# kevlar-dev/kevlar

Hardware: AMD Instinct MI355X
Metric: reads/sec through count+novel (3 samples, k=31) (higher is better)
Workload: dtype u64 hash / u8 counters

## Files before the change

__graft_entry__.py:

```python
import os
import subprocess
import sys

ROOT = os.path.dirname(os.path.abspath(__file__))
CSRC = os.path.join(ROOT, 'kevlar_amd', 'csrc')
HIP_SOURCES = ['kv_host.hip', 'kv_fastx.hip', 'kv_kernels.hip', 'kv_binned.hip', 'kv_skm.hip', 'kv_novel.hip', 'kv_graph.hip', 'kv_shard.hip', 'kv_inflate.hip', 'kv_gunzip.hip', 'kv_fastq.hip', 'kv_augfastx.hip', 'kv_synth.hip']
HIP_HEADERS = ['kv_internal.h', 'kv_knobs.h', 'kv_fastmod.h', 'kv_device.h', 'kv_binned.h', 'kv_skm_device.h', 'kv_novel_device.h', 'kv_kmer2bit_device.h', 'kv_inflate_device.h',
               os.path.join('..', '..', 'include', 'kvsketch.h')]
LIB = os.path.join(ROOT, 'kevlar_amd', 'libkvsketch_hip.so')


def _stale(target, deps):
    if not os.path.exists(target):
        return True
    t = os.path.getmtime(target)
    return any(os.path.getmtime(d) > t for d in deps)


def _compile(srcs, headers, lib, force=False, extra=()):
    from concurrent.futures import ThreadPoolExecutor
    hipcc = os.environ.get('HIPCC', '/opt/rocm/bin/hipcc')
    tag = ''.join(c if c.isalnum() else '_' for c in ' '.join(extra))
    objdir = os.path.join(CSRC, 'build', tag or 'default')
    os.makedirs(objdir, exist_ok=True)
# ... 83 lines not shown
```

kevlar_amd/csrc/kv_host.hip:

```cpp
#include <algorithm>
#include <functional>
#include <atomic>
#include <cstdarg>
#include <map>

#include "kv_internal.h"

static thread_local char g_err[512] = "";
thread_local int kv_last_hip_code = 0;

void kv_set_error(const char *fmt, ...)
{
    va_list ap;
    va_start(ap, fmt);
    vsnprintf(g_err, sizeof(g_err), fmt, ap);
    va_end(ap);
}

uint64_t kv_next_uid()
{
    static std::atomic<uint64_t> next{1};
    return next.fetch_add(1);
}

// ... 1114 lines not shown
    {"KV_COUNT_PATH", T_, "atomic | binned | skm: pin the count path"},
    {"KV_NOVEL_PATH", T_, "tiles | skm: pin the scan path"},
    {"KV_ROUTE_PATH", T_, "plain: the exchange routes one item per k-mer (no combining)"},
    {"KV_SET_SCAN", T_, "skm: a shard's set scan keeps the bucketed kernel"},
    {"KV_BIN_2BIT", T_, "0: stage A never hashes from the 2-bit form"},
    {"KV_SKM_S2", T_, "plain | sorted: pin the fine split"},
    {"KV_SKM_ANY_K", T_, "use the kernels with k at run time, not the k = 31 / 51 instances"},
    {"KV_SKM_BUCKET_KMERS", T_, "k-mer occurrences aimed at per bucket (tests: many buckets on small inputs)"},
    {"KV_SKM_CAP_PCT", T_, "segment capacity in per cent of the estimate (tests: push records through the loose list)"},
    {"KV_SKM_LOOSE_CAP", T_, "entries of the loose list"},
    {"KV_SKM_FORCE_LOOSE", T_, "one key in 64 is counted as if its table were full: its occurrences travel through the loose list"},
    {"KV_SKM_DL", T_, "0: no distinct list from a case sample's count; 1: from the first batch on"},
    {"KV_SKM_NO_REUSE", T_, "the scan re-buckets the batch instead of reusing the count's buckets"},
    {"KV_NOVEL_2BIT", T_, "0: the per-k-mer scan keeps the tile kernel"},
    {"KV_NOVEL_BITS", T_, "0: no bit map as the first probe of the scan"},
    {"KV_NOVEL_BITS_MIN", T_, "items from which the pairs scan builds its bit map"},
    {"KV_NOVEL_PAIRS", T_, "0: the set scan answers from hashes alone"},
    {"KV_NOVEL_REREAD", T_, "`kevlar novel` reads a case file again for the scan instead of keeping its batch"},
    {"KV_HOST_SORT", T_, "partition sorts its keys on the host"},
    {"KV_STAGE", T_, "0: uploads straight from the file mapping, no pinned staging"},
    {"KV_INGEST_TEXT_MB", T_, "text per ingest batch in MB (tests: small batches)"},
    {"KV_GUNZIP_TEXT_MIN_MB", T_, "gzip files from this size on are inflated on the device"},
    {"KV_GUNZIP_CHUNK_KB", T_, "1..64: compressed bytes per probe stretch"},
    {"KV_MEX_PASSES", T_, "exchange: combine passes per bucket, at least (1-16)"},
    {"KV_MEX_DL_POOL", T_, "exchange: 1 = the owner's distinct list as a pool of chunks at once (it is the last resort of an owner short of memory)"},
    {"KV_MEX_PAIRS", T_, "9: (hash, count) pairs travel in the 9-byte block form"},
    {"KV_MEX_TEST_DECLINE", T_, "point:rank -- that rank fails at that point of the exchange (tests of the agreed fallbacks)"},
    {"KV_ALLBANDS_TEST_FAIL", T_, "rank:band -- `novel --all-bands`: that rank fails before counting that band (0-based; test of the agreed stop)"},
    {"KV_ROUTE_OVF_CAP", T_, "entries of the route's overflow list (tests: force the capacity error)"},
};
// ... 56 lines not shown
```

kevlar_amd/csrc/kv_internal.h:

```cpp
#pragma once
#include <hip/hip_runtime.h>

#include <cstdint>
#include <cstdio>
#include <cstdlib>
#include <cstring>
#include <functional>
#include <atomic>
#include <mutex>
#include <string>
#include <vector>
#include "kv_knobs.h"

#include "../../include/kvsketch.h"
#include "kv_fastmod.h"

enum { ST_BYTE = 0, ST_NIBBLE = 1, ST_BIT = 2 };
enum { HF_MURMUR = 0, HF_TWOBIT = 1 };

static inline int kv_storage_of(int kind)
{
    switch (kind) {
    case KV_COUNTTABLE: case KV_COUNTGRAPH: return ST_BYTE;
    case KV_SMALLCOUNTTABLE: case KV_SMALLCOUNTGRAPH: return ST_NIBBLE;
// ... 155 lines not shown
    uint64_t band_lo, band_hi;
    int use_mask, threshold, consume_masked;
};

bool kv_binned_eligible(const kv_sketch *s, const kv_reads *reads, uint64_t n_kmers, int nbands);
int kv_consume_binned(kv_sketch *s, const kv_reads *reads, const uint64_t *d_list, uint32_t list_stride,
                      const ConsumeFilter &filter, const kv_sketch *mask, uint64_t n_kmers, int nbands, uint64_t *n_added,
                      bool weighted_list = false);
double kv_estimate_distinct(uint64_t occupied, uint64_t size);

struct NovelParams;
bool kv_skm_eligible(const kv_sketch *s, const kv_reads *reads, uint64_t n_kmers, bool for_scan);
bool kv_skm_eligible_kind(int hashfam, int ksize, const kv_reads *reads, uint64_t n_kmers, bool for_scan);
int kv_consume_skm(kv_sketch *s, const kv_reads *reads, const ConsumeFilter &filter, const kv_sketch *mask,
                   uint64_t n_kmers, int nbands, uint64_t *n_added);
int kv_skm_novel_mark(const kv_reads *reads, const NovelParams &p, uint64_t n_kmers);
void kv_tile_hits_launch(const kv_reads *reads, const NovelParams &p, hipStream_t st);
bool kv_skm_list_ready(const kv_reads *reads, int ksize);

struct KvRouteSink {
    int ndest;
    uint32_t nwg;
    uint64_t bs;
    uint64_t seg_cap;
    uint64_t *seg;
    uint32_t *seg_count;
    uint64_t *ovf;
    uint8_t *ovf_dest;
    uint64_t ovf_cap;
    unsigned long long *ctr;
};
// ... 140 lines not shown
```

kevlar_amd/csrc/kv_novel.hip:

```cpp
#include <algorithm>
#include <functional>
#include <map>

#include "kv_binned.h"
#include "kv_novel_device.h"
#include "kv_kmer2bit_device.h"

namespace {

#define VC_WINDOW 3
#define VC_WINDOW_MAX 9
__device__ __forceinline__ uint32_t kmer_minimizer_key(const uint32_t *__restrict__ words, uint32_t pos, int k, int window)
{
    const uint32_t w0 = pos >> 4, sh = 2u * (pos & 15u);
    const uint64_t lo = (uint64_t)words[w0] | ((uint64_t)words[w0 + 1] << 32);
    uint64_t code = lo >> sh;
    if (sh) code |= (uint64_t)words[w0 + 2] << (64u - sh);
    const uint64_t kmask = k == 32 ? ~0ull : ((1ull << (2 * k)) - 1ull);
    code &= kmask;
    uint64_t rev = __brevll(code);
    rev = ((rev >> 1) & 0x5555555555555555ull) | ((rev & 0x5555555555555555ull) << 1);
    rev = (~rev >> (64 - 2 * k)) & kmask;
    const int m = k - (window - 1);
    const uint64_t mmask = (1ull << (2 * m)) - 1ull;
// ... 360 lines not shown
    load_descs(ns, p);
    __syncthreads();
    const int S = p.ncase + p.nctrl, k = p.hp.k;
    const uint32_t uni_wpr = (rd.uni_len + 15u) >> 4;
    for (uint64_t i = blockIdx.x * 256ull + threadIdx.x; i < nhits; i += (uint64_t)gridDim.x * 256ull) {
        const uint32_t read = p.hit_read[i], off = p.hit_off[i];
        const uint32_t *words = rd.words + (rd.uni_len ? (uint64_t)read * uni_wpr : rd.woff[read]);
        uint64_t bw[2] = {skm_bases32(words, off), KW == 2 ? skm_bases32(words, off + 32u) : 0ull};
        const SkmKey<KW> f = skm_first_kmer<KW>(bw, k);
        const uint64_t h = skm_key_hash<KW>(f, lut, p.hp);
        if (p.ab_keys && ab_lookup(p, h, p.hit_abund + i * (uint64_t)S, S)) continue;
        hit_abundances(ns, p, h, p.hit_abund + i * (uint64_t)S);
    }
}

struct VerdictCache {
    unsigned long long *p = nullptr;
    int bits = 0;
    uint64_t signature = 0;
};
std::map<hipStream_t, VerdictCache> g_vcache;
std::mutex g_vcache_mu;

struct DevBuf {
    void *p = nullptr;
    ~DevBuf() { if (p) (void)hipFree(p); }
    hipError_t alloc(size_t n) { return kv_hip_malloc(&p, n ? n : 4); }
    template <typename T> T *as() { return (T *)p; }
};

// ... 4 lines not shown
    {
        if (n <= bytes) return hipSuccess;
        if (p) (void)hipFree(p);
        p = nullptr; bytes = 0;
        hipError_t e = kv_hip_malloc(&p, n);
        if (e == hipSuccess) bytes = n;
        return e;
    }
};
struct ScanArenas {
    Arena work, hits, set, abund;
    std::mutex mu;
    hipStream_t copy_stream = nullptr;
    hipEvent_t kdone = nullptr, copied = nullptr;
    bool copy_pending = false;
};
thread_local bool g_hits_lazy = false;
std::map<hipStream_t, ScanArenas> g_scan_arenas;
std::mutex g_scan_arenas_mu;
inline size_t up256(size_t v) { return (v + 255) & ~(size_t)255; }

int attach_vcache(NovelParams &p, kv_sketch *const *ctrls, int ncase, int nctrl, int ctrl_max, uint64_t n_kmers, hipStream_t st)
{
    if (nctrl > 0 && p.screen == 0) {
        uint64_t sig = 0x9e3779b97f4a7c15ull ^ (uint64_t)(uint32_t)ctrl_max;
        for (int c = ncase; c < ncase + nctrl; ++c) {
            const kv_sketch *sk = ctrls[c - ncase];
            sig = (sig ^ sk->uid) * 0xff51afd7ed558ccdull;
            sig = (sig ^ sk->version) * 0xc4ceb9fe1a85ec53ull;
        }
// ... 122 lines not shown
    std::lock_guard<std::mutex> arena_lock(arenas->mu);
    hipError_t e = hipSuccess;
    if (arenas->copy_pending) {
        e = hipStreamWaitEvent(st, arenas->copied, 0);
        arenas->copy_pending = false;
    }
    const uint64_t mask_words = d_mask ? 0 : (reads->n_reads * min_stride + 31) / 32;
    if (mask_words * 4 > ((uint64_t)64 << 30)) {
        kv_set_error("kv_novel_scan: %llu reads with a longest read of %u bases need a %llu GB hit mask; "
                     "scan long sequences in a batch of their own", (unsigned long long)reads->n_reads, reads->max_len,
                     (unsigned long long)(mask_words * 4 >> 30));
        delete hits;
        *out = nullptr;
        return KV_ERR_CAPACITY;
    }
    const size_t b_mask = up256(mask_words * 4), b_flags = p.screen > 0 ? up256(reads->n_reads * 4) : 0;
    const size_t b_tcount = up256((uint64_t)reads->n_tiles * 4), b_tbase = up256(((uint64_t)reads->n_tiles + 1) * 8);
    e = arenas->work.need(b_mask + b_flags + b_tcount + b_tbase + 256);
    unsigned char *wp = (unsigned char *)arenas->work.p;
    if (e == hipSuccess) {
        if (d_mask) {
            p.mask = d_mask; p.mask_stride = mask_stride;
        } else {
            p.mask_stride = min_stride;
            p.mask = (uint32_t *)wp;
            e = hipMemsetAsync(p.mask, 0, mask_words * 4, st);
        }
        wp += b_mask;
    }
    if (e == hipSuccess && p.screen > 0) {
        p.disc_first = (uint32_t *)wp;
        e = hipMemsetAsync(p.disc_first, 0xFF, reads->n_reads * 4, st);
    }
    wp += b_flags;
    p.tile_count = (uint32_t *)wp; wp += b_tcount;
    uint64_t *d_tbase_p = (uint64_t *)wp;
    p.tile_base = d_tbase_p;
    uint64_t nhits = 0;
    bool marked_by_skm = use_skm;
    p.ab_keys = nullptr; p.ab_vals = nullptr; p.ab_mask = 0; p.ab_list = nullptr; p.ab_count = nullptr; p.ab_list_cap = 0;
    if (e == hipSuccess && use_skm && !p.set_keys && kv_skm_list_ready(reads, k)) {
        uint64_t slots = 1u << 16;
        while (slots < n_kmers / 64 && slots < (1ull << 24)) slots <<= 1;
        const uint64_t list_cap = slots / 8;
        if (arenas->abund.need(up256(slots * 8) + up256(slots * (uint64_t)S) + up256(list_cap * 4) + 256) == hipSuccess) {
            p.ab_keys = (unsigned long long *)arenas->abund.p;
            p.ab_vals = (uint8_t *)arenas->abund.p + up256(slots * 8);
            p.ab_mask = slots - 1;
            p.ab_list = (uint32_t *)(p.ab_vals + up256(slots * (uint64_t)S));
            p.ab_count = (unsigned int *)((unsigned char *)p.ab_list + up256(list_cap * 4));
            p.ab_list_cap = (uint32_t)list_cap;
            e = hipMemsetAsync(p.ab_keys, 0, slots * 8, st);
            if (e == hipSuccess) e = hipMemsetAsync(p.ab_count, 0, 4, st);
        } else {
            (void)hipGetLastError();
        }
    }
    if (e == hipSuccess && use_skm) {
        const int rc = kv_skm_novel_mark(reads, p, n_kmers);
        if (rc == KV_ERR_CAPACITY) {
            marked_by_skm = false;
            if (skm_overflowed) *skm_overflowed = true;
            const int rc2 = prepare_tile_scan();
            if (rc2 != KV_OK) { delete hits; *out = nullptr; return rc2; }
        } else if (rc != KV_OK) {
            delete hits;
            *out = nullptr;
            return rc;
        }
    }
    if (e == hipSuccess) {
        const char *forced = kv_knob("KV_NOVEL_PATH"), *nm2 = kv_knob("KV_NOVEL_2BIT");
        const bool two_bit = !marked_by_skm && p.screen == 0 && fam == HF_MURMUR && k >= SKM_MIN_K && k <= SKM_MAX_K && reads->uni_len >= (uint32_t)k &&
                             reads->uni_per_tile != 0 && !(forced && strcmp(forced, "tiles") == 0) && !(nm2 && atoi(nm2) == 0);
        if (two_bit) {
            {
                KvProfScope prof("k_novel_mark_2bit");
                const uint64_t n_items = reads->n_reads * (((uint64_t)reads->uni_len - (uint64_t)k + 1 + NM2_CH - 1) / NM2_CH);
                const unsigned grid = (unsigned)std::min<uint64_t>((n_items + NM2_THREADS - 1) / NM2_THREADS, 3u * (unsigned)kv_device_cus() * 4u);
                if (k == 31 && !kv_knob("KV_SKM_ANY_K")) hipLaunchKernelGGL((k_novel_mark_2bit<1, 31>), dim3(grid), dim3(NM2_THREADS), 0, st, reads_dev(reads), p);
                else if (k <= 32) hipLaunchKernelGGL(k_novel_mark_2bit<1>, dim3(grid), dim3(NM2_THREADS), 0, st, reads_dev(reads), p);
                else hipLaunchKernelGGL(k_novel_mark_2bit<2>, dim3(grid), dim3(NM2_THREADS), 0, st, reads_dev(reads), p);
            }
            kv_tile_hits_launch(reads, p, st);
        } else if (!marked_by_skm) {
            KvProfScope prof("k_novel_mark");
            kv_ensure_dynamic_lds((const void *)k_novel_mark, reads->tile_lds_bytes);
            hipLaunchKernelGGL(k_novel_mark, dim3(reads->n_tiles), dim3(KV_TILE_THREADS), reads->tile_lds_bytes, st, reads_dev(reads), p);
        }
        {
            KvProfScope prof("k_tile_scan");
            hipLaunchKernelGGL(k_tile_scan, dim3(1), dim3(1024), 0, st, p.tile_count, reads->n_tiles, d_tbase_p);
        }
        e = hipGetLastError();
    }
    if (e == hipSuccess) e = hipMemcpyAsync(&nhits, d_tbase_p + reads->n_tiles, 8, hipMemcpyDeviceToHost, st);
    if (e == hipSuccess) e = hipStreamSynchronize(st);
    if (e == hipSuccess && nhits) {
        e = arenas->hits.need(2 * up256(nhits * 4) + up256(nhits * (uint64_t)S));
        p.hit_read = (uint32_t *)arenas->hits.p;
        p.hit_off = (uint32_t *)((unsigned char *)arenas->hits.p + up256(nhits * 4));
        p.hit_abund = (uint8_t *)arenas->hits.p + 2 * up256(nhits * 4);
        if (e == hipSuccess) {
            KvProfScope prof("k_novel_emit");
            const bool from_bits = fam == HF_MURMUR && k <= 64;
            const bool dense = from_bits && k >= SKM_MIN_K;
            const unsigned grid_hits = (unsigned)std::min<uint64_t>((nhits + 255) / 256, 1u << 16);
            if (dense && k <= 32) {
                hipLaunchKernelGGL((k_novel_emit_bits<8, false>), dim3(reads->n_tiles), dim3(256), 0, st, reads_dev(reads), p);
                hipLaunchKernelGGL(k_hit_abund<1>, dim3(grid_hits), dim3(256), 0, st, reads_dev(reads), p, nhits);
            } else if (dense) {
                hipLaunchKernelGGL((k_novel_emit_bits<16, false>), dim3(reads->n_tiles), dim3(256), 0, st, reads_dev(reads), p);
                hipLaunchKernelGGL(k_hit_abund<2>, dim3(grid_hits), dim3(256), 0, st, reads_dev(reads), p, nhits);
            } else if (from_bits) {
                hipLaunchKernelGGL((k_novel_emit_bits<8, true>), dim3(reads->n_tiles), dim3(256), 0, st, reads_dev(reads), p);
            } else {
                kv_ensure_dynamic_lds((const void *)k_novel_emit, reads->tile_lds_bytes);
                hipLaunchKernelGGL(k_novel_emit, dim3(reads->n_tiles), dim3(KV_TILE_THREADS), reads->tile_lds_bytes, st, reads_dev(reads), p);
// ... 50 lines not shown
            const uint32_t trip = first_trip[hits->read[i]];
            if (trip != 0xffffffffu) {
                if (hits->offset[i] < trip) { hits->shadow_read.push_back(hits->read[i]); hits->shadow_offset.push_back(hits->offset[i]); }
                continue;
            }
            hits->read[w] = hits->read[i];
            hits->offset[w] = hits->offset[i];
            if (w != i) memmove(&hits->abund[w * (uint64_t)S], &hits->abund[i * (uint64_t)S], (size_t)S);
            ++w;
        }
        hits->read.n = w; hits->offset.n = w; hits->abund.n = w * (uint64_t)S;
    }
    return KV_OK;
}

}

extern "C" int kv_hits_lazy(int on)
{
    g_hits_lazy = on != 0;
    return KV_OK;
}

extern "C" int kv_hits_shadow(const kv_hits *h, const uint32_t **read, const uint32_t **offset, uint64_t *n)
{
    KV_REQUIRE(h && n, KV_ERR_ARG, "kv_hits_shadow: null argument");
    h->wait();
    *n = h->shadow_read.size();
    if (read) *read = h->shadow_read.data();
    if (offset) *offset = h->shadow_offset.data();
// ... 338 lines not shown
```

kevlar_amd/csrc/kv_novel_device.h:

```cpp
#pragma once
#include "kv_device.h"
#include "kv_skm_device.h"

struct NovelParams {
    HashParams hp;
    int ncase, nctrl;
    const SketchDev *sk[KV_MAX_SAMPLES];
    int case_min, ctrl_max, screen;
    int band_mode, nbands, band;
    uint64_t band_lo, band_hi;
    uint64_t first_read;
    uint32_t *disc_first;
    uint32_t *mask;
    uint64_t mask_stride;
    uint32_t *tile_count;
    const uint64_t *tile_base;
    uint32_t *hit_read, *hit_off;
    uint8_t *hit_abund;
    unsigned long long *vcache;
    int vcache_shift;
    int vcache_sets;
    uint32_t vcache_set_mask;
    int vcache_window;
    int vcache_2bit;
    const unsigned long long *set_keys;
    const uint8_t *set_abund;
    uint64_t set_mask;
    unsigned long long *ab_keys;
    uint8_t *ab_vals;
    uint64_t ab_mask;
    uint32_t *ab_list;
    unsigned int *ab_count;
    uint32_t ab_list_cap;
    const void *host_ctrls;
    int host_nctrl;
    const void *host_case0;
    const uint32_t *case0_bits;
};
#define KV_SET_NONE 0xffffffffffffffffull

struct ProbeDesc {
    uint64_t size, magic;
    const uint8_t *tab;
};
struct NovelShared {
    ProbeDesc d[KV_MAX_SAMPLES * KV_MAX_TABLES];
    int ntab[KV_MAX_SAMPLES];
    int storage[KV_MAX_SAMPLES];
// ... 234 lines not shown
```

kevlar_amd/csrc/kv_skm.hip:

```cpp
#include <algorithm>
#include <cmath>

#include "kv_binned.h"
#include "kv_novel_device.h"
#include "kv_skm_device.h"

struct SkmGeom {
    int k, m, w, wpow;
    int kw, nbw, recw, ncap;
    uint32_t C1, F2, fbits;
    uint32_t nwg1, nwg2, quota1;
    uint32_t cap1, cap2;
    uint32_t np_max;
    uint64_t stride;
    uint64_t *seg1; uint32_t *cnt1;
    uint64_t *seg2; uint32_t *cnt2;
    uint64_t *loose; uint64_t loose_cap;
    unsigned long long *ctr;
    uint32_t n_buckets, quota3;
    uint32_t sbw;
    uint64_t bucket_kmers;
    uint32_t force_loose;
    uint64_t *abl_keys; uint8_t *abl_cnts; uint32_t *abl_bstart, *abl_bcount; uint32_t abl_cap_wg;
    uint64_t *dl_keys, *dl_hash; uint32_t *dl_bstart, *dl_bcount; uint32_t dl_cap_wg;
// ... 1510 lines not shown
        }
    }
    __syncthreads();
    if (threadIdx.x < (uint32_t)rs.ndest && dcount[threadIdx.x]) atomicAdd(&rs.ctr[ROUTE_CTR_DEST0 + threadIdx.x], (unsigned long long)dcount[threadIdx.x]);
}

__device__ __forceinline__ void skm_mark(const NovelParams &p, const ReadsDev &rd, uint64_t pos, uint64_t stride)
{
    const uint64_t read = pos / stride;
    const uint64_t off = pos - read * stride;
    if ((rd.flags[read] & 1) || read < p.first_read) return;
    const uint64_t bit = read * p.mask_stride + off;
    atomicOr(&p.mask[bit >> 5], 1u << (bit & 31));
}

template <int KW, int TS>
__global__ __launch_bounds__(SKM_THREADS3, 6) void k_skm_novel(SkmGeom sg, ReadsDev rd, NovelParams p, SkmAblSet abls)
{
    __shared__ SkmTable<KW, TS> tb;
    __shared__ uint32_t flag[TS / 32];
    __shared__ uint32_t rej[TS / 32];
    __shared__ NovelShared ns;
    __shared__ uint32_t next_bucket, any_hit;
    extern __shared__ __attribute__((aligned(16))) uint32_t dyn[];
    uint32_t *lut = dyn, *scratch = dyn + 256;
    if (threadIdx.x < 256) lut[threadIdx.x] = skm_ascii4(threadIdx.x);
    load_descs(ns, p);
    const int k = sg.k;
    if (threadIdx.x == 0) next_bucket = (uint32_t)atomicAdd(&sg.ctr[SKM_CTR_TICKET_SCAN], 1ull) * sg.bpt;
    for (uint32_t taken = 0; taken < sg.quota3; ++taken) {
// ... 58 lines not shown
        uint32_t out = 0;
        if (w * 32 + 32 <= size) {
            const uint4 a = ((const uint4 *)tab)[2 * w], b = ((const uint4 *)tab)[2 * w + 1];
            const uint32_t q[8] = {a.x, a.y, a.z, a.w, b.x, b.y, b.z, b.w};
#pragma unroll
            for (int i = 0; i < 8; ++i)
#pragma unroll
                for (int j = 0; j < 4; ++j) out |= ((int)((q[i] >> (8 * j)) & 0xffu) >= case_min ? 1u : 0u) << (4 * i + j);
        } else {
            for (uint64_t j = w * 32; j < size; ++j) out |= ((int)tab[j] >= case_min ? 1u : 0u) << (uint32_t)(j - w * 32);
        }
        bits[w] = out;
    }
}

template <int KW, int TSM>
__global__ __launch_bounds__(SKM_THREADS3, 6) void k_skm_novel_list(SkmGeom sg, ReadsDev rd, NovelParams p, SkmAblSet abls)
{
    constexpr uint32_t E = 4;
    __shared__ SkmTable<KW, TSM> rtb;
    __shared__ SkmTable<KW, TSM> itb;
    __shared__ NovelShared ns;
    __shared__ uint16_t cand[SKM_LIST_MAX];
    __shared__ uint32_t next_bucket, n_int, n_cand;
    extern __shared__ __attribute__((aligned(16))) uint32_t dyn[];
    uint32_t *scratch = dyn;
    load_descs(ns, p);
    skm_table_clear(itb);
    if (threadIdx.x == 0) { next_bucket = (uint32_t)atomicAdd(&sg.ctr[SKM_CTR_TICKET_SCAN], 1ull) * sg.bpt; n_int = 0; n_cand = 0; }
    auto mark_pass = [&](uint32_t b) {
        skm_walk_bucket<KW, true, 0, false>(sg, b, scratch, [&](const SkmKey<KW> &c, uint64_t pos) {
            if (skm_cacheable<KW>(c) && skm_table_find(itb, c) >= 0) skm_mark(p, rd, pos, sg.stride);
            return false;
        });
        __syncthreads();
        skm_table_clear(itb);
        if (threadIdx.x == 0) n_int = 0;
        __syncthreads();
    };
    for (uint32_t taken = 0; taken < sg.quota3; ++taken) {
        __syncthreads();
        const uint32_t b = next_bucket;
        if (b >= sg.n_buckets) break;
        skm_table_clear(rtb);
        __syncthreads();
        if (threadIdx.x == 0) {
            if ((b + 1u) & (sg.bpt - 1u)) next_bucket = b + 1u;
            else if (taken + 1 >= sg.quota3 || __hip_atomic_load(&sg.ctr[SKM_CTR_FAIL], __ATOMIC_RELAXED, __HIP_MEMORY_SCOPE_AGENT) != 0) next_bucket = 0xffffffffu;
            else next_bucket = (uint32_t)atomicAdd(&sg.ctr[SKM_CTR_TICKET_SCAN], 1ull) * sg.bpt;
// ... 35 lines not shown
                    const uint64_t bin = fastmod(h[u], ns.d[0].size, ns.d[0].magic);
                    const __attribute__((address_space(1))) uint32_t *bits = (const __attribute__((address_space(1))) uint32_t *)p.case0_bits;
                    v[u] = live[u] && ((bits[bin >> 5] >> (uint32_t)(bin & 31u)) & 1u) ? (uint32_t)p.case_min : 0u;
                } else {
                    v[u] = live[u] ? probe(ns, 0, 0, h[u]) : 0u;
                }
            }
#pragma unroll
            for (uint32_t u = 0; u < E; ++u)
                if (live[u] && (int)v[u] >= p.case_min) cand[atomicAdd(&n_cand, 1u)] = (uint16_t)(e0 + u * SKM_THREADS3 + threadIdx.x);
        }
        __syncthreads();
        const uint32_t nc = n_cand;
        for (uint32_t j0 = 0; j0 < nc; j0 += SKM_THREADS3) {
            const uint32_t j = j0 + threadIdx.x;
            if (j < nc) {
                const uint32_t i = cand[j];
                SkmKey<KW> c;
                c.w[0] = sg.dl_keys[(uint64_t)(e0 + i) * KW];
                if (KW == 2) c.w[KW - 1] = sg.dl_keys[(uint64_t)(e0 + i) * KW + (KW - 1)];
                const uint64_t h = sg.dl_hash[e0 + i];
                if (novel_test_wide(ns, p, h)) {
                    if (skm_table_insert(itb, c) < 0) sg.ctr[SKM_CTR_FAIL] = 1;
                    atomicAdd(&n_int, 1u);
                    if (p.ab_keys) (void)ab_claim(p, h, p.ncase + p.nctrl);
                }
            }
            __syncthreads();
            if (n_int > TSM / 4 && j0 + SKM_THREADS3 < nc) mark_pass(b);
        }
        if (n_int != 0) mark_pass(b);
    }
}

__global__ __launch_bounds__(256) void k_ab_fill(NovelParams p)
{
    __shared__ NovelShared ns;
    load_descs(ns, p);
    __syncthreads();
    const int S = p.ncase + p.nctrl;
// ... 12 lines not shown
}

template <int KW>
__global__ __launch_bounds__(256) void k_skm_loose_novel(SkmGeom sg, ReadsDev rd, NovelParams p)
{
    __shared__ uint32_t lut[256];
    __shared__ NovelShared ns;
    lut[threadIdx.x] = skm_ascii4(threadIdx.x);
    load_descs(ns, p);
    __syncthreads();
    unsigned long long n = sg.ctr[SKM_CTR_LOOSE];
    if (n > sg.loose_cap) n = sg.loose_cap;
    const int k = sg.k, recw = sg.lrecw;
    const uint32_t lane = threadIdx.x & 63u;
    auto test_one = [&](const SkmKey<KW> &fw, bool live, uint64_t pos) {
        if (!live) return;
        const uint64_t h = skm_key_hash<KW>(skm_canonical<KW>(fw, skm_revcomp<KW>(fw, k)), lut, p.hp);
        if (band_pass(p, h) && novel_test_fast(ns, p, h, nullptr, 0ull)) skm_mark(p, rd, pos, sg.stride);
    };
    const uint64_t total_waves = (uint64_t)gridDim.x * (blockDim.x >> 6), wave_id = (uint64_t)blockIdx.x * (blockDim.x >> 6) + (threadIdx.x >> 6);
    const uint32_t per = (uint32_t)min((unsigned long long)64, max((unsigned long long)1, (n + total_waves - 1) / total_waves));
    for (uint64_t i0 = wave_id * per; i0 < n; i0 += total_waves * per) {
        const uint64_t i = i0 + lane;
        const bool have = lane < per && i < n;
        const uint64_t *rec = sg.loose + (have ? i : 0) * (uint64_t)recw;
        uint64_t bw[3];
#pragma unroll
        for (int t = 0; t < 3; ++t) bw[t] = (have && t < sg.nbw) ? rec[1 + t] : 0ull;
        const uint64_t hdr = have ? rec[0] : 0ull;
        const uint32_t nk = have ? skm_hdr_n(hdr) : 0u;
        test_one(skm_first_kmer<KW>(bw, k), nk == 1, skm_hdr_pos_of(hdr, 0u));
        unsigned long long longer = __ballot(nk > 1);
        while (longer) {
// ... 692 lines not shown
    KvProfScope prof("k_case_bits");
    hipLaunchKernelGGL(k_case_bits, dim3(4096), dim3(256), 0, st, d_table, size, case_min, d_bits);
}

void kv_tile_hits_launch(const kv_reads *reads, const NovelParams &p, hipStream_t st)
{
    KvProfScope prof("k_tile_hits");
    hipLaunchKernelGGL(k_tile_hits, dim3(reads->n_tiles), dim3(64), 0, st, reads_dev(reads), p);
}

bool kv_skm_list_ready(const kv_reads *reads, int ksize)
{
    if (kv_knob("KV_SKM_NO_REUSE") || (kv_knob("KV_SKM_DL") && atoi(kv_knob("KV_SKM_DL")) == 0)) return false;
    std::lock_guard<std::mutex> lk(g_skm_mu);
    for (auto &kv : g_skm)
        if (kv.second.valid && kv.second.dl_valid && kv.second.reads_uid == reads->uid && kv.second.k == ksize) return true;
    return false;
}

int kv_skm_novel_mark(const kv_reads *reads, const NovelParams &p, uint64_t n_kmers)
{
    hipStream_t st = kv_stream();
    const int k = p.hp.k;
    SkmIndex *idx = nullptr;
    {
        std::lock_guard<std::mutex> lk(g_skm_mu);
        for (auto &kv : g_skm)
            if (kv.second.valid && kv.second.reads_uid == reads->uid && kv.second.k == k) { idx = &kv.second; break; }
        if (!idx) idx = &g_skm[kv_stream_key(st)];
    }
    std::lock_guard<std::mutex> lk(idx->mu);
    const bool reuse = idx->valid && idx->reads_uid == reads->uid && idx->k == k && !idx->g.compact && !kv_knob("KV_SKM_NO_REUSE");
    if (!reuse) {
        double hint;
        { std::lock_guard<std::mutex> glk(g_skm_mu); hint = g_skm_last_distinct; }
        const int rc = skm_build(*idx, reads, k, n_kmers, st, hint);
        if (rc != KV_OK) return rc;
    }
    SkmGeom &sg = idx->g;
    const bool from_list = reuse && idx->dl_valid && !p.set_keys && !(kv_knob("KV_SKM_DL") && atoi(kv_knob("KV_SKM_DL")) == 0);
    if (reuse) {
        if (!from_list) KV_HIP(hipMemcpyAsync(&sg.ctr[SKM_CTR_LOOSE], &sg.ctr[SKM_CTR_LOOSE_S12], 8, hipMemcpyDeviceToDevice, st));
        KV_HIP(hipMemsetAsync(&sg.ctr[SKM_CTR_TICKET_SCAN], 0, 8, st));
    }
    const uint32_t nwg3 = skm_nwg3(sg);
    const ReadsDev rd = reads_dev(reads);
    SkmAblSet abls;
    memset(&abls, 0, sizeof(abls));
    abls.ctrl_max = p.ctrl_max;
    if (p.host_ctrls && !p.set_keys) {
        const kv_sketch *const *ctrls = (const kv_sketch *const *)p.host_ctrls;
        for (int c = 0; c < p.host_nctrl && abls.n < SKM_MAX_ABL; ++c) {
            const KvAbundList &al = ctrls[c]->abl;
            if (!al.valid || al.k != k || al.m != sg.m || al.C1 != sg.C1 || al.F2 != sg.F2 || al.n_buckets != sg.n_buckets) continue;
            const int a = abls.n++;
// ... 7 lines not shown
    pl.case0_bits = nullptr;
    if (from_list && p.host_case0 && !(kv_knob("KV_NOVEL_BITS") && atoi(kv_knob("KV_NOVEL_BITS")) == 0)) {
        const kv_sketch *c0 = (const kv_sketch *)p.host_case0;
        if (c0->h.storage == ST_BYTE && !c0->lazy_zero && idx->bits.need(kv_round_up(((c0->h.size[0] + 31) >> 5) * 4, 256)) == hipSuccess) {
            kv_case_bits_launch((const uint8_t *)c0->h.tab[0], (uint64_t)c0->h.size[0], p.case_min, (uint32_t *)idx->bits.p, st);
            pl.case0_bits = (const uint32_t *)idx->bits.p;
        } else {
            (void)hipGetLastError();
        }
    }
    if (from_list) {
        KvProfScope prof("k_skm_novel_list");
        idx->list.attach(sg);
        const size_t lds = (size_t)(SKM_THREADS3 / 64) * skm_wave_scratch_words(sg.sbw) * 4;
        void (*kernel)(SkmGeom, ReadsDev, NovelParams, SkmAblSet) =
            sg.kw == 1 ? k_skm_novel_list<1, 2048> : k_skm_novel_list<2, 1024>;
        hipLaunchKernelGGL(kernel, dim3(nwg3), dim3(SKM_THREADS3), lds, st, sg, rd, pl, abls);
        if (p.ab_keys) hipLaunchKernelGGL(k_ab_fill, dim3(2048), dim3(256), 0, st, p);
        if (p.ab_list && kv_knob("KV_SKM_VERBOSE")) {
            unsigned int claimed = 0;
            if (hipMemcpyAsync(&claimed, p.ab_count, 4, hipMemcpyDeviceToHost, st) == hipSuccess && hipStreamSynchronize(st) == hipSuccess)
                fprintf(stderr, "[kv_skm] scan: %u interesting k-mers hold a slot for their abundances (the list takes %u)\n", claimed, p.ab_list_cap);
        }
        SkmDistinctList::detach(sg);
    } else {
        KvProfScope prof("k_skm_novel");
        const size_t lds = (256 + (size_t)(SKM_THREADS3 / 64) * skm_wave_scratch_words(sg.sbw)) * 4;
        if (sg.kw == 1) hipLaunchKernelGGL((k_skm_novel<1, 4096>), dim3(nwg3), dim3(SKM_THREADS3), lds, st, sg, rd, p, abls);
        else hipLaunchKernelGGL((k_skm_novel<2, 2048>), dim3(nwg3), dim3(SKM_THREADS3), lds, st, sg, rd, p, abls);
    }
    {
        KvProfScope prof("k_skm_loose_novel");
        skm_launch_loose(k_skm_loose_novel<1>, k_skm_loose_novel<2>, st, sg, rd, p);
    }
    kv_tile_hits_launch(reads, p, st);
    KV_HIP(hipGetLastError());
    unsigned long long sctr[SKM_CTR_FAIL + 1] = {0, 0};
    KV_HIP(hipMemcpyAsync(sctr, sg.ctr, sizeof(sctr), hipMemcpyDeviceToHost, st));
    KV_HIP(hipStreamSynchronize(st));
    idx->drop(SkmIndex::BATCH | SkmIndex::LIST);
    if (sctr[SKM_CTR_FAIL] != 0) {
        kv_set_error("super-k-mer scan: loose record list overflow (%llu records)", sctr[SKM_CTR_LOOSE]);
        return KV_ERR_CAPACITY;
    }
    return KV_OK;
}

static void skm_launch_route(void (*kernel)(SkmGeom, HashParams, KvRouteSink), const SkmGeom &g, int k, const KvRouteSink &rs, hipStream_t st);

int kv_skm_route_distinct(const kv_reads *reads, int ksize, uint64_t n_kmers, int ndest,
                          int (*alloc)(void *ctx, uint32_t nwg, KvRouteSink *sink), void *ctx)
{
    KV_REQUIRE(ndest >= 1 && ndest <= SKM_ROUTE_MAX_DEST, KV_ERR_ARG, "kv_skm_route_distinct: 1..%d destinations", SKM_ROUTE_MAX_DEST);
// ... 336 lines not shown
```

Before: 1.021 billion.

## Emit novel hits as a compact sorted hit list instead of marking a mask

When the scan runs from the count pass's distinct list, interesting k-mer positions are appended to a global hit list through LDS staging and wave-aggregated atomics. Abundances are looked up once per distinct interesting k-mer instead of once per occurrence. The list is then radix-sorted by position and unpacked into the hit arrays. This drops the mask memset, the mask marking, the tile-count and prefix pass, and the emit pass. It adds a rocprim sort and a fallback that re-runs the mask path when the list capacity overflows.

```diff
diff --git a/__graft_entry__.py b/__graft_entry__.py
--- a/__graft_entry__.py
+++ b/__graft_entry__.py
@@ -5,7 +5,7 @@
 ROOT = os.path.dirname(os.path.abspath(__file__))
 CSRC = os.path.join(ROOT, 'kevlar_amd', 'csrc')
 HIP_SOURCES = ['kv_host.hip', 'kv_fastx.hip', 'kv_kernels.hip', 'kv_binned.hip', 'kv_skm.hip', 'kv_novel.hip', 'kv_graph.hip', 'kv_shard.hip', 'kv_inflate.hip', 'kv_gunzip.hip', 'kv_fastq.hip', 'kv_augfastx.hip', 'kv_synth.hip']
-HIP_HEADERS = ['kv_internal.h', 'kv_knobs.h', 'kv_fastmod.h', 'kv_device.h', 'kv_binned.h', 'kv_skm_device.h', 'kv_novel_device.h', 'kv_kmer2bit_device.h', 'kv_inflate_device.h',
+HIP_HEADERS = ['kv_internal.h', 'kv_knobs.h', 'kv_fastmod.h', 'kv_device.h', 'kv_binned.h', 'kv_skm_device.h', 'kv_novel_device.h', 'kv_kmer2bit_device.h', 'kv_inflate_device.h', 'kv_hitlist.h',
                os.path.join('..', '..', 'include', 'kvsketch.h')]
 LIB = os.path.join(ROOT, 'kevlar_amd', 'libkvsketch_hip.so')
 
diff --git a/kevlar_amd/csrc/kv_hitlist.h b/kevlar_amd/csrc/kv_hitlist.h
--- /dev/null
+++ b/kevlar_amd/csrc/kv_hitlist.h
@@ -0,0 +1,50 @@
+#pragma once
+#include <stddef.h>
+#include <stdint.h>
+
+#define KV_HL_IDX_BITS 24
+#define KV_HL_POS_BITS 40
+
+struct KvHitListPlan {
+    uint64_t cap;
+    uint64_t ab_cap;
+    int pos_bits;
+    size_t off_ctr;
+    size_t off_keys, off_sorted;
+    size_t off_ab_hash;
+    size_t off_ab_vals;
+    size_t bytes;
+};
+
+static inline size_t kv_hl_up256(size_t v) { return (v + 255) & ~(size_t)255; }
+
+static inline bool kv_hitlist_plan(uint64_t n_positions, uint64_t n_kmers, uint64_t prev_hits, uint64_t forced_cap, int nsamples, KvHitListPlan *out)
+{
+    if (n_positions == 0 || n_positions > ((uint64_t)1 << KV_HL_POS_BITS) || nsamples < 1 || !out) return false;
+    uint64_t cap;
+    if (forced_cap) {
+        cap = forced_cap;
+    } else {
+        cap = n_kmers / 64;
+        const uint64_t again = prev_hits > UINT64_MAX / 2 ? UINT64_MAX : prev_hits + prev_hits / 2;
+        if (cap < again) cap = again;
+        if (cap < 4096) cap = 4096;
+    }
+    if (cap > n_positions) cap = n_positions;
+    uint64_t ab_cap = cap / 4;
+    if (ab_cap < 1024) ab_cap = 1024;
+    if (ab_cap > ((uint64_t)1 << KV_HL_IDX_BITS)) ab_cap = (uint64_t)1 << KV_HL_IDX_BITS;
+    int bits = 1;
+    while (bits < KV_HL_POS_BITS && ((uint64_t)1 << bits) < n_positions) ++bits;
+    out->cap = cap;
+    out->ab_cap = ab_cap;
+    out->pos_bits = bits;
+    size_t at = 0;
+    out->off_ctr = at;      at += 256;
+    out->off_keys = at;     at += kv_hl_up256((size_t)cap * 8);
+    out->off_sorted = at;   at += kv_hl_up256((size_t)cap * 8);
+    out->off_ab_hash = at;  at += kv_hl_up256((size_t)ab_cap * 8);
+    out->off_ab_vals = at;  at += kv_hl_up256((size_t)ab_cap * (size_t)nsamples);
+    out->bytes = at;
+    return true;
+}
diff --git a/kevlar_amd/csrc/kv_host.hip b/kevlar_amd/csrc/kv_host.hip
--- a/kevlar_amd/csrc/kv_host.hip
+++ b/kevlar_amd/csrc/kv_host.hip
@@ -1152,6 +1152,7 @@
     {"KV_SKM_NO_REUSE", T_, "the scan re-buckets the batch instead of reusing the count's buckets"},
     {"KV_NOVEL_2BIT", T_, "0: the per-k-mer scan keeps the tile kernel"},
     {"KV_NOVEL_BITS", T_, "0: no bit map as the first probe of the scan"},
+    {"KV_NOVEL_HITLIST", T_, "0: the scan from the distinct list marks the mask and takes the mask tail; N > 1: its hit list takes N entries"},
     {"KV_NOVEL_BITS_MIN", T_, "items from which the pairs scan builds its bit map"},
     {"KV_NOVEL_PAIRS", T_, "0: the set scan answers from hashes alone"},
     {"KV_NOVEL_REREAD", T_, "`kevlar novel` reads a case file again for the scan instead of keeping its batch"},
diff --git a/kevlar_amd/csrc/kv_internal.h b/kevlar_amd/csrc/kv_internal.h
--- a/kevlar_amd/csrc/kv_internal.h
+++ b/kevlar_amd/csrc/kv_internal.h
@@ -193,7 +193,8 @@
 bool kv_skm_eligible_kind(int hashfam, int ksize, const kv_reads *reads, uint64_t n_kmers, bool for_scan);
 int kv_consume_skm(kv_sketch *s, const kv_reads *reads, const ConsumeFilter &filter, const kv_sketch *mask,
                    uint64_t n_kmers, int nbands, uint64_t *n_added);
-int kv_skm_novel_mark(const kv_reads *reads, const NovelParams &p, uint64_t n_kmers);
+int kv_skm_novel_mark(const kv_reads *reads, const NovelParams &p, uint64_t n_kmers, unsigned long long *hl_counts = nullptr);
+void kv_novel_abund_launch(const NovelParams &p, hipStream_t st);
 void kv_tile_hits_launch(const kv_reads *reads, const NovelParams &p, hipStream_t st);
 bool kv_skm_list_ready(const kv_reads *reads, int ksize);
 
diff --git a/kevlar_amd/csrc/kv_novel.hip b/kevlar_amd/csrc/kv_novel.hip
--- a/kevlar_amd/csrc/kv_novel.hip
+++ b/kevlar_amd/csrc/kv_novel.hip
@@ -1,6 +1,8 @@
 #include <algorithm>
 #include <functional>
 #include <map>
+
+#include <rocprim/device/device_radix_sort.hpp>
 
 #include "kv_binned.h"
 #include "kv_novel_device.h"
@@ -398,6 +400,30 @@
     }
 }
 
+__global__ __launch_bounds__(256) void k_novel_abund(NovelParams p)
+{
+    __shared__ NovelShared ns;
+    load_descs(ns, p);
+    __syncthreads();
+    const int S = p.ncase + p.nctrl;
+    const uint64_t n = min((uint64_t)p.hl_ctr[1], (uint64_t)p.hl_ab_cap);
+    for (uint64_t i = blockIdx.x * 256ull + threadIdx.x; i < n; i += (uint64_t)gridDim.x * 256ull)
+        hit_abundances(ns, p, (uint64_t)p.hl_ab_hash[i], p.hl_ab_vals + i * (uint64_t)S);
+}
+
+__global__ __launch_bounds__(256) void k_novel_unpack(NovelParams p, const unsigned long long *__restrict__ sorted, uint64_t nhits)
+{
+    const int S = p.ncase + p.nctrl;
+    for (uint64_t i = blockIdx.x * 256ull + threadIdx.x; i < nhits; i += (uint64_t)gridDim.x * 256ull) {
+        const unsigned long long key = sorted[i];
+        const uint64_t pos = key >> KV_HL_IDX_BITS, ix = key & ((1ull << KV_HL_IDX_BITS) - 1ull);
+        const uint64_t read = pos / p.mask_stride;
+        p.hit_read[i] = (uint32_t)read;
+        p.hit_off[i] = (uint32_t)(pos - read * p.mask_stride);
+        for (int c = 0; c < S; ++c) p.hit_abund[i * (uint64_t)S + c] = p.hl_ab_vals[ix * (uint64_t)S + c];
+    }
+}
+
 struct VerdictCache {
     unsigned long long *p = nullptr;
     int bits = 0;
@@ -432,6 +458,7 @@
     hipStream_t copy_stream = nullptr;
     hipEvent_t kdone = nullptr, copied = nullptr;
     bool copy_pending = false;
+    uint64_t last_hits = 0;
 };
 thread_local bool g_hits_lazy = false;
 std::map<hipStream_t, ScanArenas> g_scan_arenas;
@@ -584,6 +611,11 @@
         *out = nullptr;
         return KV_ERR_CAPACITY;
     }
+    KvHitListPlan hl;
+    const char *hl_knob = kv_knob("KV_NOVEL_HITLIST");
+    const uint64_t hl_forced = hl_knob ? strtoull(hl_knob, nullptr, 10) : 1;
+    bool listing = use_skm && !d_mask && !p.set_keys && p.screen == 0 && p.band_mode == KV_BAND_NONE && hl_forced != 0 && kv_skm_list_ready(reads, k) &&
+                   kv_hitlist_plan(reads->n_reads * min_stride, n_kmers, arenas->last_hits, hl_forced > 1 ? hl_forced : 0, S, &hl);
     const size_t b_mask = up256(mask_words * 4), b_flags = p.screen > 0 ? up256(reads->n_reads * 4) : 0;
     const size_t b_tcount = up256((uint64_t)reads->n_tiles * 4), b_tbase = up256(((uint64_t)reads->n_tiles + 1) * 8);
     e = arenas->work.need(b_mask + b_flags + b_tcount + b_tbase + 256);
@@ -594,7 +626,7 @@
         } else {
             p.mask_stride = min_stride;
             p.mask = (uint32_t *)wp;
-            e = hipMemsetAsync(p.mask, 0, mask_words * 4, st);
+            if (!listing) e = hipMemsetAsync(p.mask, 0, mask_words * 4, st);
         }
         wp += b_mask;
     }
@@ -609,7 +641,24 @@
     uint64_t nhits = 0;
     bool marked_by_skm = use_skm;
     p.ab_keys = nullptr; p.ab_vals = nullptr; p.ab_mask = 0; p.ab_list = nullptr; p.ab_count = nullptr; p.ab_list_cap = 0;
-    if (e == hipSuccess && use_skm && !p.set_keys && kv_skm_list_ready(reads, k)) {
+    unsigned long long hl_counts[2] = {0, 0};
+    if (e == hipSuccess && listing) {
+        if (arenas->abund.need(hl.bytes) == hipSuccess) {
+            unsigned char *ap = (unsigned char *)arenas->abund.p;
+            p.hl_ctr = (unsigned long long *)(ap + hl.off_ctr);
+            p.hl_keys = (unsigned long long *)(ap + hl.off_keys);
+            p.hl_cap = hl.cap;
+            p.hl_ab_hash = (unsigned long long *)(ap + hl.off_ab_hash);
+            p.hl_ab_vals = ap + hl.off_ab_vals;
+            p.hl_ab_cap = (uint32_t)hl.ab_cap;
+            e = hipMemsetAsync(p.hl_ctr, 0, 16, st);
+        } else {
+            (void)hipGetLastError();
+            listing = false;
+            e = hipMemsetAsync(p.mask, 0, mask_words * 4, st);
+        }
+    }
+    if (e == hipSuccess && !listing && use_skm && !p.set_keys && kv_skm_list_ready(reads, k)) {
         uint64_t slots = 1u << 16;
         while (slots < n_kmers / 64 && slots < (1ull << 24)) slots <<= 1;
         const uint64_t list_cap = slots / 8;
@@ -627,8 +676,19 @@
         }
     }
     if (e == hipSuccess && use_skm) {
-        const int rc = kv_skm_novel_mark(reads, p, n_kmers);
-        if (rc == KV_ERR_CAPACITY) {
+        const int rc = kv_skm_novel_mark(reads, p, n_kmers, hl_counts);
+        if (listing && (rc == KV_ERR_CAPACITY || (rc == KV_OK && (hl_counts[0] > hl.cap || hl_counts[1] > hl.ab_cap)))) {
+            if (rc == KV_OK && hl_counts[0] != ~0ull) arenas->last_hits = hl_counts[0];
+            if (kv_knob("KV_SKM_VERBOSE")) fprintf(stderr, "[kv_novel] the hit list ran over (%llu hits for %llu, %llu k-mers for %llu): mask path\n",
+                                                   hl_counts[0], (unsigned long long)hl.cap, hl_counts[1], (unsigned long long)hl.ab_cap);
+            listing = false;
+            p.hl_keys = nullptr;
+            marked_by_skm = false;
+            if (rc == KV_ERR_CAPACITY && skm_overflowed) *skm_overflowed = true;
+            e = hipMemsetAsync(p.mask, 0, mask_words * 4, st);
+            const int rc2 = prepare_tile_scan();
+            if (rc2 != KV_OK) { delete hits; *out = nullptr; return rc2; }
+        } else if (rc == KV_ERR_CAPACITY) {
             marked_by_skm = false;
             if (skm_overflowed) *skm_overflowed = true;
             const int rc2 = prepare_tile_scan();
@@ -639,7 +699,10 @@
             return rc;
         }
     }
-    if (e == hipSuccess) {
+    if (e == hipSuccess && listing) {
+        nhits = hl_counts[0];
+        arenas->last_hits = nhits;
+    } else if (e == hipSuccess) {
         const char *forced = kv_knob("KV_NOVEL_PATH"), *nm2 = kv_knob("KV_NOVEL_2BIT");
         const bool two_bit = !marked_by_skm && p.screen == 0 && fam == HF_MURMUR && k >= SKM_MIN_K && k <= SKM_MAX_K && reads->uni_len >= (uint32_t)k &&
                              reads->uni_per_tile != 0 && !(forced && strcmp(forced, "tiles") == 0) && !(nm2 && atoi(nm2) == 0);
@@ -664,14 +727,30 @@
         }
         e = hipGetLastError();
     }
-    if (e == hipSuccess) e = hipMemcpyAsync(&nhits, d_tbase_p + reads->n_tiles, 8, hipMemcpyDeviceToHost, st);
-    if (e == hipSuccess) e = hipStreamSynchronize(st);
+    if (e == hipSuccess && !listing) e = hipMemcpyAsync(&nhits, d_tbase_p + reads->n_tiles, 8, hipMemcpyDeviceToHost, st);
+    if (e == hipSuccess && !listing) e = hipStreamSynchronize(st);
     if (e == hipSuccess && nhits) {
-        e = arenas->hits.need(2 * up256(nhits * 4) + up256(nhits * (uint64_t)S));
+        unsigned long long *hl_sorted = listing ? (unsigned long long *)((unsigned char *)arenas->abund.p + hl.off_sorted) : nullptr;
+        size_t sort_bytes = 0;
+        if (listing) e = rocprim::radix_sort_keys(nullptr, sort_bytes, p.hl_keys, hl_sorted, (size_t)nhits, KV_HL_IDX_BITS, KV_HL_IDX_BITS + hl.pos_bits, st);
+        const size_t b_arrays = 2 * up256(nhits * 4) + up256(nhits * (uint64_t)S);
+        if (e == hipSuccess) e = arenas->hits.need(b_arrays + up256(sort_bytes));
         p.hit_read = (uint32_t *)arenas->hits.p;
         p.hit_off = (uint32_t *)((unsigned char *)arenas->hits.p + up256(nhits * 4));
         p.hit_abund = (uint8_t *)arenas->hits.p + 2 * up256(nhits * 4);
-        if (e == hipSuccess) {
+        if (e == hipSuccess && listing) {
+            {
+                KvProfScope prof("k_novel_sort");
+                e = rocprim::radix_sort_keys((unsigned char *)arenas->hits.p + b_arrays, sort_bytes, p.hl_keys, hl_sorted, (size_t)nhits, KV_HL_IDX_BITS,
+                                             KV_HL_IDX_BITS + hl.pos_bits, st);
+            }
+            if (e == hipSuccess) {
+                KvProfScope prof("k_novel_unpack");
+                const unsigned grid_hits = (unsigned)std::min<uint64_t>((nhits + 255) / 256, 1u << 16);
+                hipLaunchKernelGGL(k_novel_unpack, dim3(grid_hits), dim3(256), 0, st, p, hl_sorted, nhits);
+                e = hipGetLastError();
+            }
+        } else if (e == hipSuccess) {
             KvProfScope prof("k_novel_emit");
             const bool from_bits = fam == HF_MURMUR && k <= 64;
             const bool dense = from_bits && k >= SKM_MIN_K;
@@ -752,6 +831,12 @@
     return KV_OK;
 }
 
+}
+
+void kv_novel_abund_launch(const NovelParams &p, hipStream_t st)
+{
+    KvProfScope prof("k_novel_abund");
+    hipLaunchKernelGGL(k_novel_abund, dim3(2048), dim3(256), 0, st, p);
 }
 
 extern "C" int kv_hits_lazy(int on)
diff --git a/kevlar_amd/csrc/kv_novel_device.h b/kevlar_amd/csrc/kv_novel_device.h
--- a/kevlar_amd/csrc/kv_novel_device.h
+++ b/kevlar_amd/csrc/kv_novel_device.h
@@ -1,5 +1,6 @@
 #pragma once
 #include "kv_device.h"
+#include "kv_hitlist.h"
 #include "kv_skm_device.h"
 
 struct NovelParams {
@@ -32,6 +33,12 @@
     uint32_t *ab_list;
     unsigned int *ab_count;
     uint32_t ab_list_cap;
+    unsigned long long *hl_keys;
+    unsigned long long *hl_ctr;
+    uint64_t hl_cap;
+    unsigned long long *hl_ab_hash;
+    uint8_t *hl_ab_vals;
+    uint32_t hl_ab_cap;
     const void *host_ctrls;
     int host_nctrl;
     const void *host_case0;
diff --git a/kevlar_amd/csrc/kv_skm.hip b/kevlar_amd/csrc/kv_skm.hip
--- a/kevlar_amd/csrc/kv_skm.hip
+++ b/kevlar_amd/csrc/kv_skm.hip
@@ -1548,6 +1548,19 @@
     atomicOr(&p.mask[bit >> 5], 1u << (bit & 31));
 }
 
+__device__ __forceinline__ bool skm_hit_key(const NovelParams &p, const ReadsDev &rd, uint64_t pos, uint64_t stride, uint32_t ab_index, unsigned long long &key)
+{
+    const uint64_t read = pos / stride;
+    const uint64_t off = pos - read * stride;
+    if ((rd.flags[read] & 1) || read < p.first_read) return false;
+    key = ((unsigned long long)(read * p.mask_stride + off) << KV_HL_IDX_BITS) | (unsigned long long)(ab_index & ((1u << KV_HL_IDX_BITS) - 1u));
+    return true;
+}
+__device__ __forceinline__ void skm_hit_store(const NovelParams &p, unsigned long long at, unsigned long long key)
+{
+    if (at < p.hl_cap) p.hl_keys[at] = key;
+}
+
 template <int KW, int TS>
 __global__ __launch_bounds__(SKM_THREADS3, 6) void k_skm_novel(SkmGeom sg, ReadsDev rd, NovelParams p, SkmAblSet abls)
 {
@@ -1636,7 +1649,7 @@
     }
 }
 
-template <int KW, int TSM>
+template <int KW, int TSM, bool LIST>
 __global__ __launch_bounds__(SKM_THREADS3, 6) void k_skm_novel_list(SkmGeom sg, ReadsDev rd, NovelParams p, SkmAblSet abls)
 {
     constexpr uint32_t E = 4;
@@ -1644,17 +1657,41 @@
     __shared__ SkmTable<KW, TSM> itb;
     __shared__ NovelShared ns;
     __shared__ uint16_t cand[SKM_LIST_MAX];
-    __shared__ uint32_t next_bucket, n_int, n_cand;
+    __shared__ uint32_t next_bucket, n_int, n_cand, n_hit;
+    __shared__ unsigned long long flush_base;
     extern __shared__ __attribute__((aligned(16))) uint32_t dyn[];
     uint32_t *scratch = dyn;
+    constexpr uint32_t HIT_STAGE = 1024;
+    static_assert(sizeof(SkmTable<KW, TSM>) >= HIT_STAGE * 8 + TSM * 4, "the hit stage and the abundance indices stand in rtb");
+    unsigned long long *hstage = &rtb.key[0][0];
+    uint32_t *iidx = (uint32_t *)(hstage + HIT_STAGE);
     load_descs(ns, p);
     skm_table_clear(itb);
-    if (threadIdx.x == 0) { next_bucket = (uint32_t)atomicAdd(&sg.ctr[SKM_CTR_TICKET_SCAN], 1ull) * sg.bpt; n_int = 0; n_cand = 0; }
+    if (threadIdx.x == 0) { next_bucket = (uint32_t)atomicAdd(&sg.ctr[SKM_CTR_TICKET_SCAN], 1ull) * sg.bpt; n_int = 0; n_cand = 0; n_hit = 0; }
     auto mark_pass = [&](uint32_t b) {
-        skm_walk_bucket<KW, true, 0, false>(sg, b, scratch, [&](const SkmKey<KW> &c, uint64_t pos) {
-            if (skm_cacheable<KW>(c) && skm_table_find(itb, c) >= 0) skm_mark(p, rd, pos, sg.stride);
-            return false;
-        });
+        if constexpr (LIST) {
+            skm_walk_bucket<KW, true, 0, false>(sg, b, scratch, [&](const SkmKey<KW> &c, uint64_t pos) {
+                if (!skm_cacheable<KW>(c)) return false;
+                const int at = skm_table_find(itb, c);
+                unsigned long long key;
+                if (at < 0 || !skm_hit_key(p, rd, pos, sg.stride, iidx[at], key)) return false;
+                const uint32_t i = atomicAdd(&n_hit, 1u);
+                if (i < HIT_STAGE) hstage[i] = key;
+                else skm_hit_store(p, atomicAdd(&p.hl_ctr[0], 1ull), key);
+                return false;
+            });
+            __syncthreads();
+            const uint32_t staged = min(n_hit, HIT_STAGE);
+            if (threadIdx.x == 0 && staged) flush_base = atomicAdd(&p.hl_ctr[0], (unsigned long long)staged);
+            __syncthreads();
+            for (uint32_t i = threadIdx.x; i < staged; i += SKM_THREADS3) skm_hit_store(p, flush_base + i, hstage[i]);
+            if (threadIdx.x == 0) n_hit = 0;
+        } else {
+            skm_walk_bucket<KW, true, 0, false>(sg, b, scratch, [&](const SkmKey<KW> &c, uint64_t pos) {
+                if (skm_cacheable<KW>(c) && skm_table_find(itb, c) >= 0) skm_mark(p, rd, pos, sg.stride);
+                return false;
+            });
+        }
         __syncthreads();
         skm_table_clear(itb);
         if (threadIdx.x == 0) n_int = 0;
@@ -1720,16 +1757,33 @@
         const uint32_t nc = n_cand;
         for (uint32_t j0 = 0; j0 < nc; j0 += SKM_THREADS3) {
             const uint32_t j = j0 + threadIdx.x;
+            int at = -1;
+            uint64_t h = 0;
             if (j < nc) {
                 const uint32_t i = cand[j];
                 SkmKey<KW> c;
                 c.w[0] = sg.dl_keys[(uint64_t)(e0 + i) * KW];
                 if (KW == 2) c.w[KW - 1] = sg.dl_keys[(uint64_t)(e0 + i) * KW + (KW - 1)];
-                const uint64_t h = sg.dl_hash[e0 + i];
+                h = sg.dl_hash[e0 + i];
                 if (novel_test_wide(ns, p, h)) {
-                    if (skm_table_insert(itb, c) < 0) sg.ctr[SKM_CTR_FAIL] = 1;
+                    at = skm_table_insert(itb, c);
+                    if (at < 0) sg.ctr[SKM_CTR_FAIL] = 1;
                     atomicAdd(&n_int, 1u);
-                    if (p.ab_keys) (void)ab_claim(p, h, p.ncase + p.nctrl);
+                    if (!LIST && p.ab_keys) (void)ab_claim(p, h, p.ncase + p.nctrl);
+                }
+            }
+            if constexpr (LIST) {
+                const unsigned long long found = __ballot(at >= 0);
+                if (found) {
+                    const uint32_t lane = threadIdx.x & 63u;
+                    unsigned long long first = 0;
+                    if (lane == 0) first = atomicAdd(&p.hl_ctr[1], (unsigned long long)__popcll(found));
+                    first = skm_shfl64(first, 0);
+                    if (at >= 0) {
+                        const unsigned long long ix = first + (unsigned long long)__popcll(found & ((1ull << lane) - 1ull));
+                        if (ix < p.hl_ab_cap) p.hl_ab_hash[ix] = h;
+                        iidx[at] = (uint32_t)ix;
+                    }
                 }
             }
             __syncthreads();
@@ -1772,9 +1826,32 @@
     const int k = sg.k, recw = sg.lrecw;
     const uint32_t lane = threadIdx.x & 63u;
     auto test_one = [&](const SkmKey<KW> &fw, bool live, uint64_t pos) {
-        if (!live) return;
-        const uint64_t h = skm_key_hash<KW>(skm_canonical<KW>(fw, skm_revcomp<KW>(fw, k)), lut, p.hp);
-        if (band_pass(p, h) && novel_test_fast(ns, p, h, nullptr, 0ull)) skm_mark(p, rd, pos, sg.stride);
+        uint64_t h = 0;
+        bool hit = false;
+        if (live) {
+            h = skm_key_hash<KW>(skm_canonical<KW>(fw, skm_revcomp<KW>(fw, k)), lut, p.hp);
+            hit = band_pass(p, h) && novel_test_fast(ns, p, h, nullptr, 0ull);
+        }
+        if (!p.hl_keys) {
+            if (hit) skm_mark(p, rd, pos, sg.stride);
+            return;
+        }
+        unsigned long long key = 0;
+        hit = hit && skm_hit_key(p, rd, pos, sg.stride, 0u, key);
+        const unsigned long long found = __ballot(hit);
+        if (!found) return;
+        unsigned long long first_hit = 0, first_ab = 0;
+        if (lane == 0) {
+            first_hit = atomicAdd(&p.hl_ctr[0], (unsigned long long)__popcll(found));
+            first_ab = atomicAdd(&p.hl_ctr[1], (unsigned long long)__popcll(found));
+        }
+        first_hit = skm_shfl64(first_hit, 0);
+        first_ab = skm_shfl64(first_ab, 0);
+        if (hit) {
+            const unsigned long long rank = (unsigned long long)__popcll(found & ((1ull << lane) - 1ull)), ix = first_ab + rank;
+            if (ix < p.hl_ab_cap) p.hl_ab_hash[ix] = h;
+            skm_hit_store(p, first_hit + rank, key | (ix & ((1ull << KV_HL_IDX_BITS) - 1ull)));
+        }
     };
     const uint64_t total_waves = (uint64_t)gridDim.x * (blockDim.x >> 6), wave_id = (uint64_t)blockIdx.x * (blockDim.x >> 6) + (threadIdx.x >> 6);
     const uint32_t per = (uint32_t)min((unsigned long long)64, max((unsigned long long)1, (n + total_waves - 1) / total_waves));
@@ -2497,11 +2574,11 @@
     if (kv_knob("KV_SKM_NO_REUSE") || (kv_knob("KV_SKM_DL") && atoi(kv_knob("KV_SKM_DL")) == 0)) return false;
     std::lock_guard<std::mutex> lk(g_skm_mu);
     for (auto &kv : g_skm)
-        if (kv.second.valid && kv.second.dl_valid && kv.second.reads_uid == reads->uid && kv.second.k == ksize) return true;
+        if (kv.second.valid && kv.second.dl_valid && kv.second.reads_uid == reads->uid && kv.second.k == ksize && !kv.second.g.compact) return true;
     return false;
 }
 
-int kv_skm_novel_mark(const kv_reads *reads, const NovelParams &p, uint64_t n_kmers)
+int kv_skm_novel_mark(const kv_reads *reads, const NovelParams &p, uint64_t n_kmers, unsigned long long *hl_counts)
 {
     hipStream_t st = kv_stream();
     const int k = p.hp.k;
@@ -2522,6 +2599,10 @@
     }
     SkmGeom &sg = idx->g;
     const bool from_list = reuse && idx->dl_valid && !p.set_keys && !(kv_knob("KV_SKM_DL") && atoi(kv_knob("KV_SKM_DL")) == 0);
+    if (p.hl_keys && !from_list) {
+        if (hl_counts) hl_counts[0] = hl_counts[1] = ~0ull;
+        return KV_OK;
+    }
     if (reuse) {
         if (!from_list) KV_HIP(hipMemcpyAsync(&sg.ctr[SKM_CTR_LOOSE], &sg.ctr[SKM_CTR_LOOSE_S12], 8, hipMemcpyDeviceToDevice, st));
         KV_HIP(hipMemsetAsync(&sg.ctr[SKM_CTR_TICKET_SCAN], 0, 8, st));
@@ -2559,7 +2640,8 @@
         idx->list.attach(sg);
         const size_t lds = (size_t)(SKM_THREADS3 / 64) * skm_wave_scratch_words(sg.sbw) * 4;
         void (*kernel)(SkmGeom, ReadsDev, NovelParams, SkmAblSet) =
-            sg.kw == 1 ? k_skm_novel_list<1, 2048> : k_skm_novel_list<2, 1024>;
+            p.hl_keys ? (sg.kw == 1 ? k_skm_novel_list<1, 2048, true> : k_skm_novel_list<2, 1024, true>)
+                      : (sg.kw == 1 ? k_skm_novel_list<1, 2048, false> : k_skm_novel_list<2, 1024, false>);
         hipLaunchKernelGGL(kernel, dim3(nwg3), dim3(SKM_THREADS3), lds, st, sg, rd, pl, abls);
         if (p.ab_keys) hipLaunchKernelGGL(k_ab_fill, dim3(2048), dim3(256), 0, st, p);
         if (p.ab_list && kv_knob("KV_SKM_VERBOSE")) {
@@ -2578,10 +2660,12 @@
         KvProfScope prof("k_skm_loose_novel");
         skm_launch_loose(k_skm_loose_novel<1>, k_skm_loose_novel<2>, st, sg, rd, p);
     }
-    kv_tile_hits_launch(reads, p, st);
+    if (p.hl_keys) kv_novel_abund_launch(p, st);
+    else kv_tile_hits_launch(reads, p, st);
     KV_HIP(hipGetLastError());
     unsigned long long sctr[SKM_CTR_FAIL + 1] = {0, 0};
     KV_HIP(hipMemcpyAsync(sctr, sg.ctr, sizeof(sctr), hipMemcpyDeviceToHost, st));
+    if (p.hl_keys && hl_counts) KV_HIP(hipMemcpyAsync(hl_counts, p.hl_ctr, 16, hipMemcpyDeviceToHost, st));
     KV_HIP(hipStreamSynchronize(st));
     idx->drop(SkmIndex::BATCH | SkmIndex::LIST);
     if (sctr[SKM_CTR_FAIL] != 0) {
```

Result: no change. 1.015 billion (-0.6%).
